# piotrkawa/audio-deepfake-adversarial-attacks

Measured on AMD Instinct MI355X. Metric: adversarial utterances/sec, PGD-40 LCNN+LFCC 4s@16kHz, higher is better.
Workload: dtype f32

## Files before the change

### audio_deepfake_adversarial_attacks_amd/csrc/lcnn_lstm.hip

```cpp

#include <hip/hip_runtime.h>
#include <math.h>
#include <stdint.h>
#include <stdlib.h>

#include "advstep_lcnn.h"
#include "advstep_common.h"

namespace {

__device__ __forceinline__ float sigmoidf_(float v) { return 1.0f / (1.0f + expf(-v)); }

template <int H>
__global__ __launch_bounds__(4 * H) void lstm_forward_kernel(const float *__restrict__ gx,
                                                             const float *__restrict__ w_hh, float *__restrict__ out,
                                                             float *__restrict__ gates, float *__restrict__ cell,
                                                             int T, int B, int D) {
    __shared__ __attribute__((aligned(16))) float h_s[H];
    __shared__ float pre[4 * H];
    const int b = blockIdx.x, d = blockIdx.y, j = threadIdx.x;
    float w[H];
    {
        const float *wr = w_hh + ((int64_t)d * 4 * H + j) * H;
#pragma unroll
        for (int k = 0; k < H; ++k) w[k] = wr[k];
    }
    if (j < H) h_s[j] = 0.0f;
    float c = 0.0f;
    const bool is_g = j >= 2 * H && j < 3 * H;
    __syncthreads();
    float gx_next = T > 0 ? gx[(((int64_t)(d == 0 ? 0 : T - 1) * B + b) * D + d) * 4 * H + j] : 0.0f;
    for (int step = 0; step < T; ++step) {
        const int t = d == 0 ? step : T - 1 - step;
        const int64_t row = ((int64_t)t * B + b) * D + d;
        float acc = gx_next;
        if (step + 1 < T) {
            const int tn = d == 0 ? step + 1 : T - 2 - step;
            gx_next = gx[(((int64_t)tn * B + b) * D + d) * 4 * H + j];
        }
        float a1 = 0.0f, a2 = 0.0f, a3 = 0.0f;
#pragma unroll
        for (int k = 0; k < H; k += 4) {
            const float4 hv = *reinterpret_cast<const float4 *>(&h_s[k]);
            acc = fmaf(w[k], hv.x, acc);
            a1 = fmaf(w[k + 1], hv.y, a1);
            a2 = fmaf(w[k + 2], hv.z, a2);
            a3 = fmaf(w[k + 3], hv.w, a3);
        }
        const float z = (acc + a1) + (a2 + a3);
        const float sg = 1.0f / (1.0f + expf(is_g ? -2.0f * z : -z));
        pre[j] = is_g ? 2.0f * sg - 1.0f : sg;
        lds_barrier();
        if (j < H) {
            const float ig = pre[j], fg = pre[H + j], gg = pre[2 * H + j], og = pre[3 * H + j];
            c = fg * c + ig * gg;
            const float h = og * (2.0f / (1.0f + expf(-2.0f * c)) - 1.0f);
            float *gr = gates + row * 4 * H;
            gr[j] = ig;
            gr[H + j] = fg;
            gr[2 * H + j] = gg;
            gr[3 * H + j] = og;
            cell[row * H + j] = c;
            out[((int64_t)t * B + b) * D * H + d * H + j] = h;
            h_s[j] = h;
        }
        lds_barrier();
    }
}

template <int H>
__global__ __launch_bounds__(4 * H) void lstm_backward_kernel(const float *__restrict__ dout,
                                                              const float *__restrict__ w_hh,
                                                              const float *__restrict__ gates,
                                                              const float *__restrict__ cell, float *__restrict__ dgx,
                                                              int T, int B, int D, int64_t dout_t_stride, int64_t dout_b_stride,
                                                              const float *__restrict__ dout_scale) {
    __shared__ __attribute__((aligned(16))) float dg_s[4 * H];
    __shared__ float part[4 * H];
    const int b = blockIdx.x, d = blockIdx.y, tid = threadIdx.x;
    const int k = tid % H, q = tid / H;
    float w[H];
    {
        const float *wc = w_hh + ((int64_t)d * 4 * H + (int64_t)q * H) * H + k;
#pragma unroll
        for (int jj = 0; jj < H; ++jj) w[jj] = wc[(int64_t)jj * H];
    }
    float dc_next = 0.0f;
    struct Raw {
        float ig, fg, gg, og, c, c_prev, dout;
    };
    struct Coef {
        float a_o, a_c, a_i, a_f, a_g, fg, dout;
    };
    auto load = [&](int step) {
        Raw v = {0.0f, 0.0f, 0.0f, 0.0f, 0.0f, 0.0f, 0.0f};
        if (tid < H && step >= 0) {
            const int t = d == 0 ? step : T - 1 - step, j = tid;
            const int64_t row = ((int64_t)t * B + b) * D + d;
            const float *gr = gates + row * 4 * H;
            v.ig = gr[j], v.fg = gr[H + j], v.gg = gr[2 * H + j], v.og = gr[3 * H + j];
            v.c = cell[row * H + j];
            if (step > 0) {
                const int tp = d == 0 ? step - 1 : T - step;
                v.c_prev = cell[(((int64_t)tp * B + b) * D + d) * H + j];
            }
            v.dout = dout[(int64_t)t * dout_t_stride + (int64_t)b * dout_b_stride + d * H + j];
            if (dout_scale) v.dout = dout_scale[b] * v.dout;
        }
        return v;
    };
    auto reduce = [&](const Raw &r) {
        const float tc = 2.0f / (1.0f + expf(-2.0f * r.c)) - 1.0f;
        Coef v;
        v.a_o = tc * r.og * (1.0f - r.og);
        v.a_c = r.og * (1.0f - tc * tc);
        v.a_i = r.gg * r.ig * (1.0f - r.ig);
        v.a_f = r.c_prev * r.fg * (1.0f - r.fg);
        v.a_g = r.ig * (1.0f - r.gg * r.gg);
        v.fg = r.fg;
        v.dout = r.dout;
        return v;
    };
    part[tid] = 0.0f;
    Coef cur = reduce(load(T - 1));
    Raw raw = load(T - 2);
    __syncthreads();
    for (int step = T - 1; step >= 0; --step) {
        const int t = d == 0 ? step : T - 1 - step;
        const int64_t row = ((int64_t)t * B + b) * D + d;
        if (tid < H) {
            const int j = tid;
            const float dh = cur.dout + ((part[j] + part[H + j]) + (part[2 * H + j] + part[3 * H + j]));
            const float d_o = dh * cur.a_o;
            const float dc = dh * cur.a_c + dc_next;
            const float d_i = dc * cur.a_i, d_f = dc * cur.a_f, d_g = dc * cur.a_g;
            dc_next = dc * cur.fg;
            dg_s[j] = d_i;
            dg_s[H + j] = d_f;
            dg_s[2 * H + j] = d_g;
            dg_s[3 * H + j] = d_o;
            float *dr = dgx + row * 4 * H;
            dr[j] = d_i;
            dr[H + j] = d_f;
            dr[2 * H + j] = d_g;
            dr[3 * H + j] = d_o;
        }
        lds_barrier();
        const Raw raw_next = load(step - 2);
        float4 gv[H / 4];
#pragma unroll
        for (int jj = 0; jj < H / 4; ++jj) gv[jj] = *reinterpret_cast<const float4 *>(&dg_s[q * H + 4 * jj]);
        __builtin_amdgcn_sched_barrier(0);
        f32x2 s01 = {0.0f, 0.0f}, s23 = {0.0f, 0.0f};
#pragma unroll
        for (int jj = 0; jj < H / 4; ++jj) {
            s01 = __builtin_elementwise_fma((f32x2){gv[jj].x, gv[jj].y}, (f32x2){w[4 * jj], w[4 * jj + 1]}, s01);
            s23 = __builtin_elementwise_fma((f32x2){gv[jj].z, gv[jj].w}, (f32x2){w[4 * jj + 2], w[4 * jj + 3]}, s23);
        }
        part[tid] = (s01.x + s01.y) + (s23.x + s23.y);
        const Coef nxt = reduce(raw);
        lds_barrier();
        cur = nxt;
        raw = raw_next;
    }
}



__global__ __launch_bounds__(256) void lcnn_tail_pack_kernel(const float *__restrict__ x4, float *__restrict__ xt, int B, int C,
                                                             int T, int W) {
    const int64_t total = (int64_t)T * B * C * W;
    for (int64_t i = (int64_t)blockIdx.x * blockDim.x + threadIdx.x; i < total; i += (int64_t)gridDim.x * blockDim.x) {
        const int w = (int)(i % W), c = (int)((i / W) % C), b = (int)((i / ((int64_t)W * C)) % B), t = (int)(i / ((int64_t)W * C * B));
        xt[i] = x4[(((int64_t)b * C + c) * T + t) * W + w];
    }
}

__global__ __launch_bounds__(256) void lcnn_tail_forward_kernel(const float *__restrict__ a, const float *__restrict__ xt,
                                                                const float *__restrict__ w, const float *__restrict__ bias,
                                                                float *__restrict__ z, int T, int B, int F) {
    __shared__ float red[4];
    const int b = blockIdx.x, k = threadIdx.x;
    float acc = 0.0f;
    if (k < F) {
        float s = 0.0f;
        for (int t0 = 0; t0 < T; t0 += 8) {
            float av[8], xv[8];
#pragma unroll
            for (int u = 0; u < 8; ++u) {
                const int t = t0 + u < T ? t0 + u : T - 1;
                const int64_t i = ((int64_t)t * B + b) * F + k;
                av[u] = a[i];
                xv[u] = xt[i];
            }
#pragma unroll
            for (int u = 0; u < 8; ++u)
                if (t0 + u < T) s += av[u] + xv[u];
        }
        acc = (s / (float)T) * w[k];
    }
#pragma unroll
    for (int off = 32; off > 0; off >>= 1) acc += __shfl_xor(acc, off, 64);
    if ((threadIdx.x & 63) == 0) red[threadIdx.x >> 6] = acc;
    __syncthreads();
    if (threadIdx.x == 0) z[b] = ((red[0] + red[1]) + (red[2] + red[3])) + (bias ? bias[0] : 0.0f);
}

__global__ __launch_bounds__(256) void lcnn_tail_unpack_add_kernel(const float *__restrict__ dxt, const float *__restrict__ g0,
                                                                   const float *__restrict__ dz, float *__restrict__ dx4, int B,
                                                                   int C, int T, int W) {
    const int64_t total = (int64_t)B * C * T * W;
    for (int64_t i = (int64_t)blockIdx.x * blockDim.x + threadIdx.x; i < total; i += (int64_t)gridDim.x * blockDim.x) {
        const int w = (int)(i % W), t = (int)((i / W) % T), c = (int)((i / ((int64_t)W * T)) % C), b = (int)(i / ((int64_t)W * T * C));
        const int k = c * W + w;
        const float g = dz ? dz[b] * g0[k] : g0[(int64_t)b * C * W + k];
        dx4[i] = dxt[((int64_t)t * B + b) * C * W + k] + g;
    }
}

}

extern "C" {

int advstep_lstm_supported(int64_t H) { return H == 80; }

int advstep_lstm_forward_f32(const float *gx, const float *w_hh, float *out, float *gates, float *cell, int64_t T,
                             int64_t B, int64_t D, int64_t H, advstep_stream_t stream) {
    ADVSTEP_REQUIRE(T >= 0 && B >= 0 && (D == 1 || D == 2) && advstep_lstm_supported(H));
    if (T == 0 || B == 0) return ADVSTEP_OK;
    ADVSTEP_REQUIRE(gx && w_hh && out && gates && cell && T <= INT32_MAX && B <= INT32_MAX);
    hipLaunchKernelGGL(lstm_forward_kernel<80>, dim3((unsigned)B, (unsigned)D), dim3(320), 0, as_stream(stream), gx, w_hh,
                       out, gates, cell, (int)T, (int)B, (int)D);
    return status_after_launch();
}

int advstep_lstm_backward_f32(const float *dout, const float *w_hh, const float *gates, const float *cell, float *dgx,
                              int64_t T, int64_t B, int64_t D, int64_t H, advstep_stream_t stream) {
    ADVSTEP_REQUIRE(T >= 0 && B >= 0 && (D == 1 || D == 2) && advstep_lstm_supported(H));
    if (T == 0 || B == 0) return ADVSTEP_OK;
    ADVSTEP_REQUIRE(dout && w_hh && gates && cell && dgx && T <= INT32_MAX && B <= INT32_MAX);
    hipLaunchKernelGGL(lstm_backward_kernel<80>, dim3((unsigned)B, (unsigned)D), dim3(320), 0, as_stream(stream), dout,
                       w_hh, gates, cell, dgx, (int)T, (int)B, (int)D, (int64_t)B * D * H, (int64_t)D * H,
                       static_cast<const float *>(nullptr));
    return status_after_launch();
}

int advstep_lstm_backward_bcast_f32(const float *dout_row, const float *w_hh, const float *gates, const float *cell,
                                    float *dgx, int64_t T, int64_t B, int64_t D, int64_t H, advstep_stream_t stream) {
    ADVSTEP_REQUIRE(T >= 0 && B >= 0 && (D == 1 || D == 2) && advstep_lstm_supported(H));
    if (T == 0 || B == 0) return ADVSTEP_OK;
    ADVSTEP_REQUIRE(dout_row && w_hh && gates && cell && dgx && T <= INT32_MAX && B <= INT32_MAX);
    hipLaunchKernelGGL(lstm_backward_kernel<80>, dim3((unsigned)B, (unsigned)D), dim3(320), 0, as_stream(stream), dout_row,
                       w_hh, gates, cell, dgx, (int)T, (int)B, (int)D, (int64_t)0, (int64_t)D * H, static_cast<const float *>(nullptr));
    return status_after_launch();
}

int advstep_lstm_backward_outer_f32(const float *dz, const float *row, const float *w_hh, const float *gates, const float *cell,
                                    float *dgx, int64_t T, int64_t B, int64_t D, int64_t H, advstep_stream_t stream) {
    ADVSTEP_REQUIRE(T >= 0 && B >= 0 && (D == 1 || D == 2) && advstep_lstm_supported(H));
    if (T == 0 || B == 0) return ADVSTEP_OK;
    ADVSTEP_REQUIRE(dz && row && w_hh && gates && cell && dgx && T <= INT32_MAX && B <= INT32_MAX);
    hipLaunchKernelGGL(lstm_backward_kernel<80>, dim3((unsigned)B, (unsigned)D), dim3(320), 0, as_stream(stream), row, w_hh, gates,
                       cell, dgx, (int)T, (int)B, (int)D, (int64_t)0, (int64_t)0, dz);
    return status_after_launch();
}

int advstep_lcnn_tail_pack_f32(const float *x4, float *xt, int64_t B, int64_t C, int64_t T, int64_t W, advstep_stream_t stream) {
    ADVSTEP_REQUIRE(B >= 0 && C >= 0 && T >= 0 && W >= 0);
    const int64_t total = B * C * T * W;
    if (total == 0) return ADVSTEP_OK;
    ADVSTEP_REQUIRE(x4 && xt && B <= INT32_MAX && C <= INT32_MAX && T <= INT32_MAX && W <= INT32_MAX);
    const int64_t blocks = (total + 255) / 256;
    hipLaunchKernelGGL(lcnn_tail_pack_kernel, dim3((unsigned)(blocks < 4096 ? blocks : 4096)), dim3(256), 0, as_stream(stream), x4,
                       xt, (int)B, (int)C, (int)T, (int)W);
    return status_after_launch();
}

int advstep_lcnn_tail_forward_f32(const float *a, const float *xt, const float *w, const float *bias, float *z, int64_t T,
                                  int64_t B, int64_t F, advstep_stream_t stream) {
    ADVSTEP_REQUIRE(T >= 1 && B >= 0 && F >= 1 && F <= 256);
    if (B == 0) return ADVSTEP_OK;
    ADVSTEP_REQUIRE(a && xt && w && z && T <= INT32_MAX && B <= INT32_MAX);
    hipLaunchKernelGGL(lcnn_tail_forward_kernel, dim3((unsigned)B), dim3(256), 0, as_stream(stream), a, xt, w, bias, z, (int)T,
                       (int)B, (int)F);
    return status_after_launch();
}

int advstep_lcnn_tail_unpack_add_f32(const float *dxt, const float *g0, float *dx4, int64_t B, int64_t C, int64_t T, int64_t W,
                                     advstep_stream_t stream) {
    ADVSTEP_REQUIRE(B >= 0 && C >= 0 && T >= 0 && W >= 0);
    const int64_t total = B * C * T * W;
    if (total == 0) return ADVSTEP_OK;
    ADVSTEP_REQUIRE(dxt && g0 && dx4 && B <= INT32_MAX && C <= INT32_MAX && T <= INT32_MAX && W <= INT32_MAX);
    const int64_t blocks = (total + 255) / 256;
    hipLaunchKernelGGL(lcnn_tail_unpack_add_kernel, dim3((unsigned)(blocks < 4096 ? blocks : 4096)), dim3(256), 0,
                       as_stream(stream), dxt, g0, static_cast<const float *>(nullptr), dx4, (int)B, (int)C, (int)T, (int)W);
    return status_after_launch();
}

int advstep_lcnn_tail_unpack_add_outer_f32(const float *dxt, const float *dz, const float *row, float *dx4, int64_t B, int64_t C,
                                           int64_t T, int64_t W, advstep_stream_t stream) {
    ADVSTEP_REQUIRE(B >= 0 && C >= 0 && T >= 0 && W >= 0);
    const int64_t total = B * C * T * W;
    if (total == 0) return ADVSTEP_OK;
    ADVSTEP_REQUIRE(dxt && dz && row && dx4 && B <= INT32_MAX && C <= INT32_MAX && T <= INT32_MAX && W <= INT32_MAX);
    const int64_t blocks = (total + 255) / 256;
    hipLaunchKernelGGL(lcnn_tail_unpack_add_kernel, dim3((unsigned)(blocks < 4096 ? blocks : 4096)), dim3(256), 0,
                       as_stream(stream), dxt, row, dz, dx4, (int)B, (int)C, (int)T, (int)W);
    return status_after_launch();
}

}
```

Measured before the change: 2093.

## Stage LSTM gate inputs and backward coefficients in LDS chunks of timesteps

Adds staged LSTM forward and backward kernels that load TC=8 timesteps of gx (forward) or gate/cell/dout data (backward) into shared memory in one coalesced batch. The backward kernel precomputes the per-step coefficients for the whole chunk in parallel across all threads, then writes dgx back as float4 rows. This takes per-step global loads off the serial recurrence critical path, at the cost of more LDS per block. A shared coefficient helper uses inline-asm multiplies to keep the rounding order fixed. The new kernels are the default, selected through an environment variable and a 16-byte alignment check.

```diff
diff --git a/audio_deepfake_adversarial_attacks_amd/csrc/lcnn_lstm.hip b/audio_deepfake_adversarial_attacks_amd/csrc/lcnn_lstm.hip
--- a/audio_deepfake_adversarial_attacks_amd/csrc/lcnn_lstm.hip
+++ b/audio_deepfake_adversarial_attacks_amd/csrc/lcnn_lstm.hip
@@ -10,6 +10,26 @@
 namespace {
 
 __device__ __forceinline__ float sigmoidf_(float v) { return 1.0f / (1.0f + expf(-v)); }
+
+__device__ __forceinline__ float mul_ab(float a, float b) {
+    float r;
+    asm("v_mul_f32_e32 %0, %1, %2" : "=v"(r) : "v"(a), "v"(b));
+    return r;
+}
+
+struct LstmCoef {
+    float a_i, a_f, a_g, a_o, a_c;
+};
+__device__ __forceinline__ LstmCoef lstm_coefs(float ig, float fg, float gg, float og, float c, float c_prev) {
+    const float tc = 2.0f / (1.0f + expf(-2.0f * c)) - 1.0f;
+    LstmCoef v;
+    v.a_o = mul_ab(1.0f - og, mul_ab(og, tc));
+    v.a_c = mul_ab(og, 1.0f - tc * tc);
+    v.a_i = mul_ab(mul_ab(gg, ig), 1.0f - ig);
+    v.a_f = mul_ab(mul_ab(c_prev, fg), 1.0f - fg);
+    v.a_g = mul_ab(ig, 1.0f - gg * gg);
+    return v;
+}
 
 template <int H>
 __global__ __launch_bounds__(4 * H) void lstm_forward_kernel(const float *__restrict__ gx,
@@ -110,13 +130,9 @@
         return v;
     };
     auto reduce = [&](const Raw &r) {
-        const float tc = 2.0f / (1.0f + expf(-2.0f * r.c)) - 1.0f;
+        const LstmCoef a = lstm_coefs(r.ig, r.fg, r.gg, r.og, r.c, r.c_prev);
         Coef v;
-        v.a_o = tc * r.og * (1.0f - r.og);
-        v.a_c = r.og * (1.0f - tc * tc);
-        v.a_i = r.gg * r.ig * (1.0f - r.ig);
-        v.a_f = r.c_prev * r.fg * (1.0f - r.fg);
-        v.a_g = r.ig * (1.0f - r.gg * r.gg);
+        v.a_o = a.a_o, v.a_c = a.a_c, v.a_i = a.a_i, v.a_f = a.a_f, v.a_g = a.a_g;
         v.fg = r.fg;
         v.dout = r.dout;
         return v;
@@ -166,6 +182,179 @@
 }
 
 
+constexpr int kLstmTC = 8;
+
+template <int H, int TC>
+__global__ __launch_bounds__(4 * H) void lstm_forward_staged_kernel(const float *__restrict__ gx,
+                                                                    const float *__restrict__ w_hh, float *__restrict__ out,
+                                                                    float *__restrict__ gates, float *__restrict__ cell,
+                                                                    int T, int B, int D) {
+    constexpr int SLOT = 4 * H;
+    static_assert(TC % 4 == 0, "TC * H quads of gx over 4H threads");
+    __shared__ __attribute__((aligned(16))) float stage[TC * SLOT];
+    __shared__ __attribute__((aligned(16))) float h_s[H];
+    const int b = blockIdx.x, d = blockIdx.y, j = threadIdx.x;
+    float w[H];
+    {
+        const float *wr = w_hh + ((int64_t)d * 4 * H + j) * H;
+#pragma unroll
+        for (int k = 0; k < H; ++k) w[k] = wr[k];
+    }
+    if (j < H) h_s[j] = 0.0f;
+    float c = 0.0f;
+    const bool is_g = j >= 2 * H && j < 3 * H;
+    for (int s0 = 0; s0 < T; s0 += TC) {
+        const int n = T - s0 < TC ? T - s0 : TC;
+        {
+            float4 v[TC / 4];
+#pragma unroll
+            for (int u = 0; u < TC / 4; ++u) {
+                const int e = u * 4 * H + j, i = e / H < n ? e / H : n - 1;
+                const int t = d == 0 ? s0 + i : T - 1 - (s0 + i);
+                v[u] = *reinterpret_cast<const float4 *>(gx + (((int64_t)t * B + b) * D + d) * 4 * H + 4 * (e % H));
+            }
+#pragma unroll
+            for (int u = 0; u < TC / 4; ++u) {
+                const int e = u * 4 * H + j;
+                *reinterpret_cast<float4 *>(&stage[(e / H) * SLOT + 4 * (e % H)]) = v[u];
+            }
+        }
+        __syncthreads();
+        for (int i = 0; i < n; ++i) {
+            const int t = d == 0 ? s0 + i : T - 1 - (s0 + i);
+            const int64_t row = ((int64_t)t * B + b) * D + d;
+            float *slot = stage + i * SLOT;
+            float acc = slot[j];
+            float a1 = 0.0f, a2 = 0.0f, a3 = 0.0f;
+#pragma unroll
+            for (int k = 0; k < H; k += 4) {
+                const float4 hv = *reinterpret_cast<const float4 *>(&h_s[k]);
+                acc = fmaf(w[k], hv.x, acc);
+                a1 = fmaf(w[k + 1], hv.y, a1);
+                a2 = fmaf(w[k + 2], hv.z, a2);
+                a3 = fmaf(w[k + 3], hv.w, a3);
+            }
+            const float z = (acc + a1) + (a2 + a3);
+            const float sg = 1.0f / (1.0f + expf(is_g ? -2.0f * z : -z));
+            const float act = is_g ? 2.0f * sg - 1.0f : sg;
+            slot[j] = act;
+            gates[row * 4 * H + j] = act;
+            lds_barrier();
+            if (j < H) {
+                const float ig = slot[j], fg = slot[H + j], gg = slot[2 * H + j], og = slot[3 * H + j];
+                c = fg * c + ig * gg;
+                const float h = og * (2.0f / (1.0f + expf(-2.0f * c)) - 1.0f);
+                cell[row * H + j] = c;
+                out[((int64_t)t * B + b) * D * H + d * H + j] = h;
+                h_s[j] = h;
+            }
+            lds_barrier();
+        }
+    }
+}
+
+template <int H, int TC>
+__global__ __launch_bounds__(4 * H) void lstm_backward_staged_kernel(const float *__restrict__ dout,
+                                                                     const float *__restrict__ w_hh,
+                                                                     const float *__restrict__ gates,
+                                                                     const float *__restrict__ cell, float *__restrict__ dgx,
+                                                                     int T, int B, int D, int64_t dout_t_stride,
+                                                                     int64_t dout_b_stride, const float *__restrict__ dout_scale) {
+    constexpr int SLOT = 7 * H;
+    static_assert(TC % 4 == 0 && H % 4 == 0, "TC * H items over 4H threads; rows leave as quads");
+    __shared__ __attribute__((aligned(16))) float stage[TC * SLOT];
+    __shared__ float part[4 * H];
+    const int b = blockIdx.x, d = blockIdx.y, tid = threadIdx.x;
+    const int k = tid % H, q = tid / H;
+    float w[H];
+    {
+        const float *wc = w_hh + ((int64_t)d * 4 * H + (int64_t)q * H) * H + k;
+#pragma unroll
+        for (int jj = 0; jj < H; ++jj) w[jj] = wc[(int64_t)jj * H];
+    }
+    const float scale = dout_scale ? dout_scale[b] : 0.0f;
+    const int dir = d == 0 ? 1 : -1, t_of0 = d == 0 ? 0 : T - 1;
+    float dc_next = 0.0f;
+    part[tid] = 0.0f;
+    for (int hi = T - 1; hi >= 0; hi -= TC) {
+        const int lo = hi - TC + 1 > 0 ? hi - TC + 1 : 0, n = hi - lo + 1;
+        {
+            float ig[TC / 4], fg[TC / 4], gg[TC / 4], og[TC / 4], cc[TC / 4], cp[TC / 4], dv[TC / 4];
+#pragma unroll
+            for (int u = 0; u < TC / 4; ++u) {
+                const int i = min(4 * u + q, n - 1), step = lo + i;
+                const int t = t_of0 + dir * step, tp = t - dir * min(step, 1);
+                const int64_t row = ((int64_t)t * B + b) * D + d;
+                const float *gr = gates + row * 4 * H;
+                ig[u] = gr[k], fg[u] = gr[H + k], gg[u] = gr[2 * H + k], og[u] = gr[3 * H + k];
+                cc[u] = cell[row * H + k];
+                cp[u] = cell[(((int64_t)tp * B + b) * D + d) * H + k];
+                dv[u] = dout[(int64_t)t * dout_t_stride + (int64_t)b * dout_b_stride + d * H + k];
+            }
+            asm volatile("" : "+v"(cp[0]));
+#pragma unroll
+            for (int u = 0; u < TC / 4; ++u) {
+                const float c_prev = lo + 4 * u + q > 0 ? cp[u] : 0.0f;
+                const float dval = dout_scale ? scale * dv[u] : dv[u];
+                const LstmCoef a = lstm_coefs(ig[u], fg[u], gg[u], og[u], cc[u], c_prev);
+                float *slot = stage + (4 * u + q) * SLOT + k;
+                slot[0] = a.a_i;
+                slot[H] = a.a_f;
+                slot[2 * H] = a.a_g;
+                slot[3 * H] = a.a_o;
+                slot[4 * H] = a.a_c;
+                slot[5 * H] = fg[u];
+                slot[6 * H] = dval;
+            }
+        }
+        __syncthreads();
+        float a_i = 0.0f, a_f = 0.0f, a_g = 0.0f, a_o = 0.0f, a_c = 0.0f, fgc = 0.0f, dval = 0.0f;
+        if (tid < H) {
+            const float *slot = stage + (n - 1) * SLOT + k;
+            a_i = slot[0], a_f = slot[H], a_g = slot[2 * H], a_o = slot[3 * H], a_c = slot[4 * H], fgc = slot[5 * H], dval = slot[6 * H];
+        }
+        for (int i = n - 1; i >= 0; --i) {
+            float *slot = stage + i * SLOT;
+            if (tid < H) {
+                const int j = tid;
+                const float dh = dval + ((part[j] + part[H + j]) + (part[2 * H + j] + part[3 * H + j]));
+                const float d_o = dh * a_o;
+                const float dc = dh * a_c + dc_next;
+                const float d_i = dc * a_i, d_f = dc * a_f, d_g = dc * a_g;
+                dc_next = dc * fgc;
+                slot[j] = d_i;
+                slot[H + j] = d_f;
+                slot[2 * H + j] = d_g;
+                slot[3 * H + j] = d_o;
+            }
+            lds_barrier();
+            if (tid < H) {
+                const float *nx = stage + (i > 0 ? i - 1 : 0) * SLOT + k;
+                a_i = nx[0], a_f = nx[H], a_g = nx[2 * H], a_o = nx[3 * H], a_c = nx[4 * H], fgc = nx[5 * H], dval = nx[6 * H];
+            }
+            float4 gv[H / 4];
+#pragma unroll
+            for (int jj = 0; jj < H / 4; ++jj) gv[jj] = *reinterpret_cast<const float4 *>(&slot[q * H + 4 * jj]);
+            __builtin_amdgcn_sched_barrier(0);
+            f32x2 s01 = {0.0f, 0.0f}, s23 = {0.0f, 0.0f};
+#pragma unroll
+            for (int jj = 0; jj < H / 4; ++jj) {
+                s01 = __builtin_elementwise_fma((f32x2){gv[jj].x, gv[jj].y}, (f32x2){w[4 * jj], w[4 * jj + 1]}, s01);
+                s23 = __builtin_elementwise_fma((f32x2){gv[jj].z, gv[jj].w}, (f32x2){w[4 * jj + 2], w[4 * jj + 3]}, s23);
+            }
+            part[tid] = (s01.x + s01.y) + (s23.x + s23.y);
+            lds_barrier();
+        }
+        for (int e = tid; e < n * H; e += 4 * H) {
+            const int i = e / H, t = t_of0 + dir * (lo + i);
+            *reinterpret_cast<float4 *>(dgx + (((int64_t)t * B + b) * D + d) * 4 * H + 4 * (e % H)) =
+                *reinterpret_cast<const float4 *>(&stage[i * SLOT + 4 * (e % H)]);
+        }
+        lds_barrier();
+    }
+}
+
+
 
 __global__ __launch_bounds__(256) void lcnn_tail_pack_kernel(const float *__restrict__ x4, float *__restrict__ xt, int B, int C,
                                                              int T, int W) {
@@ -218,6 +407,19 @@
     }
 }
 
+bool lstm_staged() {
+    const char *e = getenv("ADVSTEP_LSTM_STAGED");
+    return !(e && e[0] == '0');
+}
+
+void launch_lstm_backward(const float *dout, const float *w_hh, const float *gates, const float *cell, float *dgx, int64_t T,
+                          int64_t B, int64_t D, int64_t t_stride, int64_t b_stride, const float *dout_scale, hipStream_t st) {
+    const dim3 grid((unsigned)B, (unsigned)D), block(320);
+    auto kernel = lstm_staged() && aligned16(dgx) ? lstm_backward_staged_kernel<80, kLstmTC> : lstm_backward_kernel<80>;
+    hipLaunchKernelGGL(kernel, grid, block, 0, st, dout, w_hh, gates, cell, dgx, (int)T, (int)B, (int)D, t_stride, b_stride,
+                       dout_scale);
+}
+
 }
 
 extern "C" {
@@ -229,8 +431,9 @@
     ADVSTEP_REQUIRE(T >= 0 && B >= 0 && (D == 1 || D == 2) && advstep_lstm_supported(H));
     if (T == 0 || B == 0) return ADVSTEP_OK;
     ADVSTEP_REQUIRE(gx && w_hh && out && gates && cell && T <= INT32_MAX && B <= INT32_MAX);
-    hipLaunchKernelGGL(lstm_forward_kernel<80>, dim3((unsigned)B, (unsigned)D), dim3(320), 0, as_stream(stream), gx, w_hh,
-                       out, gates, cell, (int)T, (int)B, (int)D);
+    auto kernel = lstm_staged() && aligned16(gx) ? lstm_forward_staged_kernel<80, kLstmTC> : lstm_forward_kernel<80>;
+    hipLaunchKernelGGL(kernel, dim3((unsigned)B, (unsigned)D), dim3(320), 0, as_stream(stream), gx, w_hh, out, gates, cell,
+                       (int)T, (int)B, (int)D);
     return status_after_launch();
 }
 
@@ -239,9 +442,7 @@
     ADVSTEP_REQUIRE(T >= 0 && B >= 0 && (D == 1 || D == 2) && advstep_lstm_supported(H));
     if (T == 0 || B == 0) return ADVSTEP_OK;
     ADVSTEP_REQUIRE(dout && w_hh && gates && cell && dgx && T <= INT32_MAX && B <= INT32_MAX);
-    hipLaunchKernelGGL(lstm_backward_kernel<80>, dim3((unsigned)B, (unsigned)D), dim3(320), 0, as_stream(stream), dout,
-                       w_hh, gates, cell, dgx, (int)T, (int)B, (int)D, (int64_t)B * D * H, (int64_t)D * H,
-                       static_cast<const float *>(nullptr));
+    launch_lstm_backward(dout, w_hh, gates, cell, dgx, T, B, D, B * D * H, D * H, nullptr, as_stream(stream));
     return status_after_launch();
 }
 
@@ -250,8 +451,7 @@
     ADVSTEP_REQUIRE(T >= 0 && B >= 0 && (D == 1 || D == 2) && advstep_lstm_supported(H));
     if (T == 0 || B == 0) return ADVSTEP_OK;
     ADVSTEP_REQUIRE(dout_row && w_hh && gates && cell && dgx && T <= INT32_MAX && B <= INT32_MAX);
-    hipLaunchKernelGGL(lstm_backward_kernel<80>, dim3((unsigned)B, (unsigned)D), dim3(320), 0, as_stream(stream), dout_row,
-                       w_hh, gates, cell, dgx, (int)T, (int)B, (int)D, (int64_t)0, (int64_t)D * H, static_cast<const float *>(nullptr));
+    launch_lstm_backward(dout_row, w_hh, gates, cell, dgx, T, B, D, 0, D * H, nullptr, as_stream(stream));
     return status_after_launch();
 }
 
@@ -260,8 +460,7 @@
     ADVSTEP_REQUIRE(T >= 0 && B >= 0 && (D == 1 || D == 2) && advstep_lstm_supported(H));
     if (T == 0 || B == 0) return ADVSTEP_OK;
     ADVSTEP_REQUIRE(dz && row && w_hh && gates && cell && dgx && T <= INT32_MAX && B <= INT32_MAX);
-    hipLaunchKernelGGL(lstm_backward_kernel<80>, dim3((unsigned)B, (unsigned)D), dim3(320), 0, as_stream(stream), row, w_hh, gates,
-                       cell, dgx, (int)T, (int)B, (int)D, (int64_t)0, (int64_t)0, dz);
+    launch_lstm_backward(row, w_hh, gates, cell, dgx, T, B, D, 0, 0, dz, as_stream(stream));
     return status_after_launch();
 }
 
```

Result: no change. 2091 (-0.1%).
